# BhavikJoshi/skybox_rt

Measured on AMD Instinct MI355X. Metric: Mrays/sec per GPU + achieved HBM GB/s, 1024^2 primary+shadow tekkaman, higher is better.
Workload: dtype f32

## Files before the change

include/vx_rt.h:

```cpp
#ifndef VX_RT_H
#define VX_RT_H

#include <stdint.h>

#ifdef __cplusplus
extern "C" {
#endif

typedef struct rt_scene* rt_scene_h;
typedef struct rt_renderer* rt_renderer_h;

typedef struct {
  uint32_t num_drawcalls, num_prims, num_geometry, num_layer, num_textures;
  uint32_t bvh_nodes, bvh_tris, bvh_leaves, bvh_depth;
  uint32_t bvh4_nodes, bvh4_depth, bvh4_stack;
  uint32_t bvh4_f16;
  double parse_ms, bvh_ms;
} rt_scene_info_t;

#define RT_RENDER_SHADOWS 0x1u
#define RT_RENDER_PATH 0x8u
#define RT_RENDER_FLAT 0x10u
#define RT_RENDER_RASTER 0x20u
#define RT_RENDER_BVH2 0x40u
// ... 75 lines not shown
int rt_render_kernel_ms(rt_renderer_h r, double* kernel_ms);
int rt_render_run_totals(rt_renderer_h r, double* kernel_ms_sum, uint64_t* timed,
                         uint64_t* launches);
int rt_render_set_timing(rt_renderer_h r, int timed);
int rt_read_framebuffer(rt_renderer_h r, uint32_t* out, uint64_t count);
int rt_read_framebuffer_prev(rt_renderer_h r, uint32_t* out, uint64_t count);

int rt_read_depthbuffer(rt_renderer_h r, uint32_t* out, uint64_t count);

typedef struct {
  uint32_t nodes, depth, launches;
  uint32_t stack4;
  double build_ms;
  double kernel_ms;
  uint32_t nodes4;
  uint32_t depth4;
  uint32_t method;
  uint32_t pad;
} rt_bvh_build_stats_t;
int rt_renderer_build_bvh(rt_renderer_h r, rt_bvh_build_stats_t* stats);
#define RT_BVH_BUILD_LBVH 0u
#define RT_BVH_BUILD_SAH 1u
#define RT_BVH_BUILD_HOST 2u
int rt_renderer_build_bvh_ex(rt_renderer_h r, uint32_t method, rt_bvh_build_stats_t* stats);
int rt_renderer_bvh_stats(rt_renderer_h r, rt_bvh_build_stats_t* stats);
#define RT_BVH_STACK4_UNUSED 0xFFFFFFFFu
int rt_renderer_export_bvh4(rt_renderer_h r, float* nodes4, uint32_t* num_nodes4);
int rt_renderer_export_bvh4h(rt_renderer_h r, void* nodes4h, uint32_t* num_nodes4);
int rt_renderer_export_bvh(rt_renderer_h r, float* nodes, float* tris, uint32_t* num_nodes,
                           uint32_t* num_tris);

int rt_renderer_export_vis_tree(rt_renderer_h r, int32_t* refs, uint32_t* num_nodes,
                                int32_t* leaf_pids, uint32_t* num_leaf);

typedef struct {
  uint32_t device;
  uint32_t launches;
  uint32_t heavy_tiles;
  uint32_t blist_blocks;
  double setup_ms;
  double configure_ms;
  uint64_t blist_entries;
  uint32_t blist_max;
  uint32_t slist_on;
  uint64_t slist_entries;
  uint32_t path_queue;
  uint32_t slist_built;
  uint32_t slist_stale;
  uint32_t lane_grid;
  uint32_t bg_first_chunk;
  uint32_t tier_groups;
  uint64_t btrim_entries;
  uint32_t btrim_blocks;
  uint32_t pad;
} rt_setup_stats_t;
int rt_renderer_setup_stats(rt_renderer_h r, rt_setup_stats_t* stats);

int rt_renderer_set_light(rt_renderer_h r, const float light[3]);
int rt_renderer_set_list_policy(rt_renderer_h r, uint32_t defer_frames);

#define RT_MAX_LIGHTS 16u
int rt_renderer_set_lights(rt_renderer_h r, const float (*lights)[3], uint32_t n);
typedef struct {
  float light[3];
  uint32_t slist_on;
  uint64_t slist_entries;
} rt_light_info_t;
int rt_renderer_lights_info(rt_renderer_h r, rt_light_info_t* out, uint32_t max, uint32_t* n);
int rt_renderer_export_light_lists(rt_renderer_h r, uint32_t light, uint32_t which, void* out, uint64_t bytes,
                                   uint64_t* size);
uint32_t rt_lights_resolve(uint32_t argb, uint32_t occluded, uint32_t k);

#define RT_MAX_PATH_LIGHTS 8u
int rt_renderer_set_path_lights(rt_renderer_h r, const float (*lights)[3], uint32_t n);
uint32_t rt_path_lights_resolve(const uint32_t sums[3], uint32_t k, uint32_t alpha_argb);

#define RT_AOV_GEOM 0x01000000u
#define RT_AOV_SHADOW_RAY 0x02000000u
typedef struct {
  int32_t  pid;
  uint32_t depth_flags;
  float    t;
  uint32_t light_mask;
} rt_aov_t;
int rt_render_aov_start(rt_renderer_h r);
int rt_render_aov(rt_renderer_h r);
int rt_read_aov(rt_renderer_h r, rt_aov_t* out, uint64_t count);
uint32_t rt_aov_relight(uint32_t plain_argb, uint32_t light_mask, uint32_t k);

int rt_relight_capture_start(rt_renderer_h r);
int rt_relight_capture(rt_renderer_h r);
int rt_render_relight_start(rt_renderer_h r, const uint8_t* weights, uint32_t n);
int rt_render_relight(rt_renderer_h r, const uint8_t* weights, uint32_t n);
int rt_read_relight_base(rt_renderer_h r, uint32_t* out, uint64_t count);
uint32_t rt_relight_resolve(uint32_t base_argb, uint32_t depth_flags, uint32_t light_mask, const uint8_t* weights,
                            uint32_t n);

typedef struct {
  int32_t  pid;
  uint32_t depth_flags;
  uint32_t normal;
  uint32_t reserved;
} rt_denoise_guide_t;
typedef struct {
  uint32_t passes;
  uint32_t depth_shift;
  uint32_t color_shift;
// ... 53 lines not shown
```

skybox_rt_amd/csrc/app/rt_app.cpp:

```cpp
#include <dlfcn.h>

#include <algorithm>
#include <cstdio>
#include <cstdlib>
#include <chrono>
#include <map>
#include <cstring>
#include <memory>
#include <string>
#include <vector>

#include "VX_types.h"
#include "app_util.h"
#include "bg_tier.h"
#include "bvh.h"
#include "bvh_common.h"
#include "cgltrace.h"
#include "rt_internal.h"
#include "sah_common.h"
#include "setup_common.h"
#include "setup.h"
#include "vis.h"
#include "vortex.h"
#include "rt_shard.h"
#include "vortex_hip.h"
#include "vx_rt.h"

namespace {

thread_local std::string g_err;

int fail(const std::string& m, int code = -1) {
  g_err = m;
  return code;
}

std::string find_lib_dir() {
  Dl_info info;
  if (dladdr((void*)&find_lib_dir, &info) && info.dli_fname) {
    std::string p(info.dli_fname);
    auto pos = p.rfind('/');
    if (pos != std::string::npos) return p.substr(0, pos);
  }
  return ".";
}

const std::string& lib_dir() {
  static const std::string dir = find_lib_dir();
  return dir;
}

bool file_exists(const std::string& path) {
  FILE* f = std::fopen(path.c_str(), "rb");
  if (f) std::fclose(f);
  return f != nullptr;
}

int upload_image(rt_renderer* r, const std::string& path, vx_buffer_h* out) {
  if (vx_upload_kernel_file(r->dev, path.c_str(), out) == 0) return 0;
  *out = nullptr;
  return fail("cannot upload kernel " + path);
}

int release_idle(rt_renderer* r, vx_buffer_h* buf) {
  if (!*buf) return 0;
  if (vx_ready_wait(r->dev, VX_MAX_TIMEOUT) != 0) return fail("vx_ready_wait failed");
  vx_mem_free(*buf);
  *buf = nullptr;
  return 0;
}
// ... 370 lines not shown
  if (leaf_pids && !r->vis_pids.empty())
    std::memcpy(leaf_pids, r->vis_pids.data(), r->vis_pids.size() * 4);
  return 0;
}

static uint32_t lane_grid_of(rt_renderer* r) {
  if (r->lane_grid_known) return r->lane_grid;
  r->lane_grid_known = true;
  r->lane_grid = 0;
  uint64_t ia = 0;
  uint32_t block = 0, mgrid = 0;
  const vx_buffer_h rt = r->img[rtimg::mode_image(0, 0, r->deep)];
  if (r->lane_chunks > 1 && rt && vx_mem_address(rt, &ia) == 0 &&
      r->launch_shape(r->dev, ia, &block, &mgrid) == 0 && block >= 64) {
    const uint32_t chunks = (r->arg.num_tasks + 63u) / 64u, per = r->lane_chunks * (block / 64u);
    const uint32_t g = std::max(1u, (chunks + per - 1u) / per);
    if (g < mgrid) r->lane_grid = g;
  }
  return r->lane_grid;
}

static uint32_t tier_groups_of(rt_renderer* r, int k, uint32_t grid, bool laned) {
  if (!r->bg_ok || r->bg_mode == 0 || (r->bg_mode == 1 && !laned)) return 0;
  if (r->sl_stale && !r->bg_stale) return 0;
  if (!r->img_shape_known[k]) {
    r->img_shape_known[k] = true;
    uint64_t ia = 0;
    const vx_buffer_h rt = r->img[rtimg::IMG_RT + k];
    if (!(r->launch_shape && rt && vx_mem_address(rt, &ia) == 0 &&
          r->launch_shape(r->dev, ia, &r->img_block[k], &r->img_grid[k]) == 0))
      r->img_block[k] = r->img_grid[k] = 0;
  }
  if (r->img_block[k] < 64 || r->img_grid[k] == 0) return 0;
  if (grid == 0 || grid > r->img_grid[k]) grid = r->img_grid[k];
  const uint32_t chunks = (r->arg.num_tasks + 63u) / 64u;
  return vxtier::tier_groups(vxtier::Config{}, chunks, r->bg_first / vxtier::kChunksPerTile, grid,
                             r->img_block[k] / 64u, r->bg_cost);
}

int rt_renderer_setup_stats(rt_renderer_h r, rt_setup_stats_t* st) {
  if (!r || !st) return fail("null argument");
  if (!r->configured) return fail("renderer not configured");
  if (rtapp::settle_lists(r) != 0) return -1;
  if (r->trim_on && !r->trim_counted) {
    uint32_t c[2] = {0, 0};
    if (vx_copy_from_dev(c, r->btrim_args, RT_BTRIM_ARG_OFFSET + offsetof(rt_btrim_arg_t, stat), sizeof(c)) != 0)
      return fail("vx_copy_from_dev failed");
    r->setup.btrim_entries = c[0];
    r->setup.btrim_blocks = c[1];
    r->trim_counted = true;
  }
  r->setup.slist_on = r->arg.slist_on;
  r->setup.slist_stale = r->sl_stale ? 1u : 0u;
  r->setup.lane_grid = lane_grid_of(r);
  r->setup.bg_first_chunk = r->bg_ok ? r->bg_first : 0u;
  {
    const int k = (r->params.flags & RT_RENDER_INSTRUMENTED) ? 1 : 0;
    r->setup.tier_groups = r->lanes ? tier_groups_of(r, k, r->sl_stale ? 0u : lane_grid_of(r), true)
                                    : tier_groups_of(r, k, 0u, false);
  }
  *st = r->setup;
  return 0;
}

int rt_renderer_set_light(rt_renderer_h r, const float light[3]) {
  if (!r || !light) return fail("null argument");
  if (!r->configured) return fail("renderer not configured");
  if (!(r->params.flags & (RT_RENDER_SHADOWS | RT_RENDER_PATH)) || (r->params.flags & RT_RENDER_RASTER))
    return fail("rt_renderer_set_light: the configuration traces no shadow rays");
  uint32_t launches = 0;
  r->nlights = 0;
  r->relight_n = 0;
  if (rtapp::set_light(r, light, &launches) != 0) return -1;
  r->setup.slist_built = r->sl_mode ? 1u : 0u;
  if (r->accum_on) {
    r->accum_reset = true;
    r->accum_n = 0;
  }
  return 0;
}


static int set_several_lights(rt_renderer_h r, const float (*lights)[3], uint32_t n, rtimg::Group group,
                              const char* who, bool lists, bool need_lists) {
  if (const int e = rtapp::load_images(r, group, who)) return e;
  if (n == 1) {
    const uint32_t defer = r->sl_defer;
    r->sl_defer = 0;
    const int e = rt_renderer_set_light(r, lights[0]);
    r->sl_defer = defer;
    if (e != 0) return e;
    return rtapp::settle_lists(r);
  }
  uint32_t launches = 0;
  if (rtapp::build_light_sets(r, lights, n, lists, &launches) != 0) return -1;
  rt_lights_arg_t la{};
  la.count = n;
  la.slist_n = r->arg.slist_n;
  for (uint32_t i = 0; i < n; ++i) {
    const LightSet& l = r->lsets[i];
    if (need_lists && !l.built)
      return fail(std::string(who) + ": the light-space lists of light " + std::to_string(i) +
                  " do not fit (pt_lights has no BVH shadow walk)", -2);
    std::memcpy(la.l[i].light, l.light, sizeof(l.light));
    la.l[i].slist_on = l.built ? 1u : 0u;
    la.l[i].sidx_addr = l.sidx_addr;
// ... 716 lines not shown
    if (*b) { vx_mem_free(*b); *b = nullptr; }
  if (release_idle(r, &r->accum) != 0) return -1;
  r->accum_on = r->accum_reset = false;
  r->accum_bytes = 0;
  r->accum_n = 0;
  if (release_idle(r, &r->aov) != 0) return -1;
  r->aov_bytes = 0;
  if (release_idle(r, &r->relight_base) != 0) return -1;
  r->relight_base_bytes = 0;
  r->relight_n = 0;
  if (release_idle(r, &r->dn_buf) != 0) return -1;
  r->dn_bytes = 0;
  r->dn_captured = false;
  r->nlights = 0;
  rt_kernel_arg_t& a = r->arg;
  a.width = p->width;
  a.height = p->height;
  uint32_t tlog = RT_TILE_LOG;
  if (raster) {
    tlog = RT_RASTER_TILE_LOG;
    if (const char* e = std::getenv("RT_RASTER_TILE_LOG")) tlog = std::atoi(e) == 5 ? 5u : 4u;
  }
  a.raster_tile_log = tlog;
  a.raster_bin_log = p->tile_logsize ? p->tile_logsize : RT_TILE_LOG;
  if (raster && (a.raster_bin_log < 2 || a.raster_bin_log > 15))
    return fail("tile_logsize must be in [2, 15] (raster_unit.cpp:92)");
  if (!raster && a.raster_bin_log != RT_TILE_LOG)
    return fail("the RT modes bin at RASTER_TILE_LOGSIZE 5; other tile sizes need RT_RENDER_RASTER");
  if ((p->flags & RT_RENDER_COVERAGE) && !raster) return fail("RT_RENDER_COVERAGE needs RT_RENDER_RASTER");
  a.tiles_y = (p->height + (1u << tlog) - 1) >> tlog;
  a.tiles_x = (p->width + (1u << tlog) - 1) >> tlog;
  a.tiles_x_magic = rt_tiles_x_magic(a.tiles_x);
  const uint32_t tiles = a.tiles_x * a.tiles_y;
  r->local_tiles = (tiles > p->shard_index) ? (tiles - p->shard_index + shards - 1) / shards : 0;
  a.num_tasks = r->local_tiles * (raster ? 256u : RT_TILE_PIXELS);
  a.shard_index = p->shard_index;
  a.shard_count = shards;
  a.order_addr = 0;
  a.split_tiles = 0;
  a.split_log = 5;
  a.quad_tiles = 0;
  const bool order_on = !raster && r->local_tiles > 0 &&
                        !(std::getenv("RT_TILE_ORDER") && std::atoi(std::getenv("RT_TILE_ORDER")) == 0);
  bool use_bvh4 = !(p->flags & RT_RENDER_BVH2) && (!r->gpu_bvh || r->gpu_bvh4);
  if (const char* e = std::getenv("RT_BVH_WIDTH")) use_bvh4 = use_bvh4 && std::atoi(e) != 2;
  r->use_bvh4 = use_bvh4;
  a.flags = ((p->flags & RT_RENDER_SHADOWS) ? RT_FLAG_SHADOWS : 0u) |
            ((p->flags & RT_RENDER_PATH) ? RT_FLAG_PATH : 0u) |
            ((p->flags & RT_RENDER_FLAT) ? RT_FLAG_FLAT : 0u) |
            (raster ? RT_FLAG_RASTER : 0u) |
            ((p->flags & RT_RENDER_COVERAGE) ? RT_FLAG_COVERAGE : 0u) |
            (s->tie_high ? RT_FLAG_TIE_HIGH : 0u) | (compact ? RT_FLAG_COMPACT : 0u) |
            (use_bvh4 ? RT_FLAG_BVH4 : 0u) |
            (use_bvh4 && (r->gpu_bvh || !s->bvh.nodes4h.empty()) ? RT_FLAG_BVH4H : 0u);
  if (tail && s->geometry.size() > 0 && !(a.flags & RT_FLAG_BVH4H))
    return fail("a scene with an ordered tail needs the binary16 BVH4; this tree needs the generic (deep) "
                "images, which have no output-merger variant (use RT_RENDER_RASTER)", -2);
  if (!raster && !tail && !(p->flags & RT_RENDER_FLAT) && !(a.flags & RT_FLAG_BVH4H) && !r->deep &&
      load_deep_images(r) != 0)
    return -1;
  const char* pqe = std::getenv("RT_PT_QUEUE");
  r->pq = (p->flags & RT_RENDER_PATH) && !r->generic_tree() && r->img[rtimg::IMG_PT_PRIMARY] &&
          r->launch_group && pqe && std::atoi(pqe) == 1;
  a.bounces = p->bounces;
  a.seed = p->seed;
  a.clear_color = p->clear_color;
  a.sx = 2.0f / (float)p->width;
  a.sy = 2.0f / (float)p->height;
  a.light[0] = p->light[0];
  a.light[1] = p->light[1];
  a.light[2] = p->light[2];
  const uint64_t npx = compact ? (uint64_t)r->local_tiles * RT_TILE_PIXELS
                                  : (uint64_t)p->width * p->height;
  r->cbuf_bytes = npx * 4;
  const char* sv = std::getenv("RT_SETUP");
  const char* vt = std::getenv("RT_VIS_TREE");
  const bool device = !(p->flags & RT_RENDER_HOST_SETUP) && !(sv && std::string(sv) == "host") &&
                      !(!raster && vt && std::string(vt) == "screen");
  uint32_t heavy = 0, launches = 0;
  const char* bl = std::getenv("RT_BLOCK_LISTS");
  const bool bvh_walk = (p->flags & RT_RENDER_BVH_WALK) != 0;
  const bool lists = !raster && !(p->flags & RT_RENDER_FLAT) && !(bl && std::atoi(bl) == 0) && !bvh_walk &&
                     a.num_geom > 0 && r->local_tiles > 0;
  a.blist_blocks = 0;
  a.blist_addr = a.bidx_addr = 0;
  a.cdesc_addr = 0;
  a.cdesc_first = 0;
  r->cdesc_n = 0;
  r->setup.blist_entries = 0;
  r->setup.blist_max = 0;
  const char* bte = std::getenv("RT_BLIST_TRIM");
  const bool trim = lists && !(p->flags & RT_RENDER_INSTRUMENTED) && !(bte && std::atoi(bte) == 0);
  r->trim_on = r->trim_counted = false;
  r->setup.btrim_entries = 0;
  r->setup.btrim_blocks = 0;
  const char* sle = std::getenv("RT_SHADOW_LISTS");
  const bool slists = device && !raster && !(p->flags & RT_RENDER_FLAT) &&
                      (p->flags & (RT_RENDER_SHADOWS | RT_RENDER_PATH)) && a.num_geom > 0 &&
                      !(sle && std::atoi(sle) == 0) && !bvh_walk;
  r->sl_mode = slists;
  r->sl_stale = false;
  a.slist_on = 0;
  r->setup.slist_entries = 0;
  const auto t1 = std::chrono::steady_clock::now();
  if (device) {
    r->vis_refs.clear();
    r->vis_pids.clear();
// ... 1048 lines not shown
```

skybox_rt_amd/csrc/kernels/rt_common.h:

```cpp
#pragma once

#include <stdint.h>

#ifndef RT_BLOCK_THREADS
#define RT_BLOCK_THREADS 64
#endif
#define RT_STACK_SHALLOW 24
#define RT_STACK_DEEP 32
#ifndef RT_MAX_STACK
#define RT_MAX_STACK RT_STACK_SHALLOW
#endif
#ifndef RT_PUSH_UNCOND
#define RT_PUSH_UNCOND 0
#endif
#define RT_STACK_ROWS (RT_MAX_STACK + (RT_PUSH_UNCOND ? 3 : 0))
#define RT_TILE_LOG 5
#define RT_TILE_PIXELS 1024
#define RT_RASTER_TILE_LOG 4

#define RT_FLAG_SHADOWS  0x1u
#define RT_FLAG_TIE_HIGH 0x2u
#define RT_FLAG_COMPACT  0x4u
#define RT_FLAG_PATH     0x8u
#define RT_FLAG_FLAT     0x10u
#define RT_FLAG_RASTER   0x20u
#define RT_FLAG_BVH4     0x40u
#define RT_FLAG_BVH4H    0x80u
#define RT_FLAG_COVERAGE 0x100u

#define RT_LW_LIGHT    0x1u
#define RT_LW_NO_SLIST 0x2u
#define RT_LW_CBUF_MASK 0xffffff00u
#define RT_LW_ACCUM_RESET   0x4u
#define RT_LW_ACCUM_K_SHIFT 3
#define RT_LW_ACCUM_K_MASK  0xf8u
#define RT_ACCUM_MAX_K      32u
#define RT_ACCUM_MAX_SAMPLES (1u << 24)

#define RT_DC_DEPTH   0x1u
#define RT_DC_COLOR   0x2u
#define RT_DC_TEX     0x4u
#define RT_DC_MODULATE 0x8u

#define RT_LEAF_FLAG 0x80000000u
#define RT_EMPTY_REF (-1)

#define RT_MPM_USER 3
enum {
  RT_STAT_PRIMARY = 0, RT_STAT_SHADOW, RT_STAT_HITS, RT_STAT_OCCLUDED,
  RT_STAT_NODE_VISITS, RT_STAT_TRI_TESTS, RT_STAT_LAYER_TESTS, RT_STAT_SHADED,
  RT_STAT_TEXEL_BYTES, RT_STAT_BOUNCE, RT_STAT_RECT_TESTS, RT_STAT_EDGE_TESTS, RT_STAT_COUNT = 16
};

typedef struct { float v[16]; } rt_node_t;

typedef struct { float v[32]; } rt_node4_t;

typedef struct { uint16_t b[24]; int32_t child[4]; } rt_node4h_t;


typedef struct { float v[12]; } rt_tri_t;

#define RT_VIS_EMPTY_RECT 0x0000ffffu
#define RT_VIS_ZMIN_NONE 0xffffffffu
typedef struct {
  uint32_t lo[4], hi[4], zmin[4];
  int32_t child[4];
} rt_vnode_t;
typedef struct {
  int32_t edges[9];
  uint32_t rx, ry;
  int32_t pid;
  int32_t z[3];
  uint32_t zmin;
} rt_vtri_t;

typedef struct {
  int32_t edges[3][3];
  int32_t attribs[7][3];
  uint32_t dc;
  uint32_t pad;
// ... 260 lines not shown
```

skybox_rt_amd/csrc/kernels/rt_kernel.hip:

```cpp
#include <hip/hip_runtime.h>

#ifndef RT_BLOCK_THREADS
#define RT_BLOCK_THREADS 64
#endif
#define VX_BLOCK_THREADS RT_BLOCK_THREADS
#include "rt_trace.h"

#ifndef RT_LIGHTS
#define RT_LIGHTS 0
#endif
#ifndef RT_PATHQ
#define RT_PATHQ 0
#endif
#ifndef RT_BG_TIER
#define RT_BG_TIER 0
#endif
#ifndef RT_BG_LAYERS
#define RT_BG_LAYERS 0
#endif
#if RT_BG_LAYERS && !RT_BG_TIER
#error "RT_BG_LAYERS is for the background tier"
#endif
#if RT_BG_LAYERS && !defined(RT_INSTRUMENT) && !RT_LIGHTS
#define RT_BG_TABLE 1
#else
#define RT_BG_TABLE 0
#endif
#if RT_LIGHTS && (RT_PATHQ || RT_BVH_WALK || !RT_ONLY_BVH4H)
#error "RT_LIGHTS is for the primary+shadow list image on the binary16 BVH4"
#endif
#if RT_BG_TIER && (RT_PATHQ || RT_BVH_WALK || !RT_CHUNK_DESC)
#error "RT_BG_TIER is for the primary+shadow list image with the chunk descriptor table"
#endif

namespace {

using namespace rtk;

constexpr int kWaves = RT_BLOCK_THREADS / 64;

#define RT_QUEUE 128
#define RT_LANE_STACK (!RT_ONLY_BVH4H)
struct WaveLds {
#if RT_LANE_STACK
  int32_t stack[RT_STACK_ROWS][64];
#define RT_WSTACK(w, lane) (&(w).stack[0][(lane)])
#else
#define RT_WSTACK(w, lane) ((int32_t*)nullptr)
#endif
  uint32_t q_out[RT_QUEUE];
  uint32_t q_xy[RT_QUEUE];
  float q_t[RT_QUEUE];
  int32_t q_pid[RT_QUEUE];
  uint32_t q_color[RT_QUEUE];
  uint32_t q_count;
};

__device__ __forceinline__ void kernel_body(const vx_task_t& task, const Scene& S, WaveLds& w,
                                            Counters& cnt) {
  const uint32_t t = task.blockIdx.x;
  const uint32_t c = (uint32_t)__builtin_amdgcn_readfirstlane(t) >> 6;
  uint32_t x, y, out;
#if RT_CHUNK_DESC && !RT_BVH_WALK
  uint2 oc = make_uint2(0u, 0u);
  if (S.cdesc != 0 && c >= S.cdesc_first) {
    const uint4 d = S.A.sld_u4(S.cdesc + 16u * (c - S.cdesc_first));
    uint32_t ln = t & 63u;
    asm volatile("" : "+v"(ln));
    x = (d.x & 0xffffu) + (ln & 7u);
    y = (d.x >> 16) + (ln >> 3);
    out = d.y + (ln >> 3) * (d.w >> 16) + (ln & 7u);
    oc = make_uint2(d.z, d.w & 0xffffu);
  } else {
    const ChunkMap cm = chunk_map(S, task_args(S), c);
    uint32_t cx, cy, co;
    chunk_pixel(S, cm, t & 63u, &cx, &cy, &co);
    x = cx;
    y = cy;
    out = co;
    if (S.blist_blocks) oc = block_header(S, (cm.lt << 4) | cm.blk);
  }
#else
  const ChunkMap cm = chunk_map(S, task_args(S), c);
  chunk_pixel(S, cm, t & 63u, &x, &y, &out);
  const uint32_t lb = (cm.lt << 4) | cm.blk;
#endif
  const bool in = x < S.width && y < S.height;
  cnt.primary += in;
  const bool tie_high = (S.flags & RT_FLAG_TIE_HIGH) != 0;
#ifdef RT_STAMPS
  if (lane_id() == 0) __vx_mpm_lds[3] = (uint32_t)__builtin_amdgcn_s_memrealtime();
#endif
#if RT_CHUNK_DESC && !RT_BVH_WALK
  int32_t hit;
  if (S.blist_blocks) {
    hit = block_primary(S, oc, x, y, in, tie_high, cnt);
  } else {
    const int32_t h = trace_primary_packet(walk_scene(S), x, y, in, tie_high, cnt);
    hit = in ? h : -1;
  }
#else
  const int32_t hit = trace_primary(S, lb, x, y, in, tie_high, cnt);
#endif
#ifdef RT_STAMPS
  if (lane_id() == 0) __vx_mpm_lds[14] = (uint32_t)__builtin_amdgcn_s_memrealtime();
#endif
  cnt.hits += hit >= 0;
  const int32_t spid = resolve_layers(S, x, y, in && hit < 0, hit, cnt);
#ifdef RT_STAMPS
  if (lane_id() == 0) __vx_mpm_lds[4] = (uint32_t)__builtin_amdgcn_s_memrealtime();
#endif
  uint32_t color = shade_wave(S, spid, x, y, S.clear_color, cnt);
#ifdef RT_STAMPS
  if (lane_id() == 0) __vx_mpm_lds[11] = (uint32_t)__builtin_amdgcn_s_memrealtime();
#endif
  Ray r;
  primary_dir(S, x, y, r);
  const float th = hit >= 0 ? plane_t(S, r, hit) : 0.0f;
#if RT_PATHQ
  const bool path = hit >= 0 && secondary_ok(th);
  pathq_append(S, path, t, th, hit, color);
  if (in && !path) store_out(S, out, color);
  (void)w;
  return;
#endif
  const bool shadow = hit >= 0 && secondary_ok(th) && (rt_usgpr(S.flags) & RT_FLAG_SHADOWS) != 0;
  const uint64_t m = __ballot(shadow);
  if (m) {
    const uint32_t base = w.q_count;
    if (shadow) {
      const uint32_t rank = __builtin_amdgcn_mbcnt_hi(
          (uint32_t)(m >> 32), __builtin_amdgcn_mbcnt_lo((uint32_t)m, 0u));
      const uint32_t slot = base + rank;
      w.q_out[slot] = out;
      w.q_xy[slot] = x | (y << 16);
      w.q_t[slot] = th;
      w.q_pid[slot] = hit;
      w.q_color[slot] = color;
    }
    __builtin_amdgcn_wave_barrier();
    if (lane_id() == 0) w.q_count = base + (uint32_t)__popcll(m);
    __builtin_amdgcn_wave_barrier();
  }
  if (in && !shadow) store_out(S, out, color);
#ifdef RT_STAMPS
  if (lane_id() == 0) __vx_mpm_lds[5] = (uint32_t)__builtin_amdgcn_s_memrealtime();
#endif
}

__device__ __forceinline__ void shadow_drain(bool final, const Scene& S, WaveLds& w,
                                             Counters& cnt) {
#ifdef RT_STAMPS
  if (final && lane_id() == 0) __vx_mpm_lds[15] = (uint32_t)__builtin_amdgcn_s_memrealtime();
  if (final && lane_id() == 0) __vx_mpm_lds[8] = w.q_count;
  if (!final && w.q_count >= 64 && lane_id() == 0)
    __vx_mpm_lds[6] = (uint32_t)__builtin_amdgcn_s_memrealtime();
#endif
  if (!(rt_usgpr(S.flags) & RT_FLAG_SHADOWS)) return;
  const uint32_t lane = lane_id();
  uint32_t n = w.q_count;
  const bool tie_high = (S.flags & RT_FLAG_TIE_HIGH) != 0;
  while (n >= 64 || (final && n > 0)) {
    const uint32_t take = n < 64 ? n : 64;
    const uint32_t base = n - take;
    const bool active = lane < take;
    const uint32_t slot = base + lane;
    const uint32_t xy = w.q_xy[slot];
// ... 112 lines not shown
#else
      const int32_t spid = resolve_layers(S, x, y, in, -1, cnt);
      const uint32_t color = shade_wave(S, spid, x, y, S.clear_color, cnt);
#endif
      if (in) store_out(S, out, color);
      ++ran;
    }
  }
  vx_mpm_add(VX_MPM_TASKS, ran);
  flush(RT_STAT_PRIMARY, cnt.primary);
#ifdef RT_INSTRUMENT
  flush(RT_STAT_LAYER_TESTS, cnt.layer_tests);
  flush(RT_STAT_SHADED, cnt.shaded);
  flush(RT_STAT_TEXEL_BYTES, cnt.texel_bytes);
#endif
}
#endif

}

#if !defined(RT_WAVES_PER_EU) && RT_ONLY_BVH4H
#if RT_BVH_WALK
#define RT_WAVES_PER_EU 5
#else
#define RT_WAVES_PER_EU 7
#endif
#endif
#ifdef RT_WAVES_PER_EU
VX_MAIN_OCC(rt_kernel_arg_t, arg, RT_BLOCK_THREADS, RT_WAVES_PER_EU) {
#else
VX_MAIN(rt_kernel_arg_t, arg, RT_BLOCK_THREADS) {
#endif
#if RT_BG_TIER
  if (vx_launch_tag != 0 && blockIdx.x >= vx_launch_tag) {
    bg_tier(arg, vx_launch_tag, vx_launch_words);
    return 0;
  }
#endif
  __shared__ WaveLds s_wave[kWaves];
  WaveLds& w = s_wave[threadIdx.x >> 6];
#ifdef RT_STAMPS
  const uint64_t t_stamp0 = __builtin_amdgcn_s_memrealtime();
#endif
  Counters cnt;
  Scene S = load_scene(arg, vx_launch_words);
#ifdef RT_STAMPS
  if (threadIdx.x == 0) __vx_mpm_lds[10] = (uint32_t)__builtin_amdgcn_s_memrealtime();
#endif
  if ((threadIdx.x & 63u) == 0) w.q_count = 0;
  __builtin_amdgcn_wave_barrier();
#if RT_BG_TIER
  const uint32_t tier_wgs = vx_launch_tag != 0 ? vx_launch_tag : gridDim.x;
  const uint32_t tier_end = vx_launch_tag != 0 ? bg_first_chunk(arg) : 0xffffffffu;
  const int rc = vx_spawn_chunks_ex(
      S.num_tasks, 0u, tier_end, blockIdx.x * kWaves + (threadIdx.x >> 6), tier_wgs * kWaves,
      [&](const vx_task_t& task, const Scene* s) { kernel_body(task, *s, w, cnt); },
      [&](bool final, const Scene* s) { shadow_drain(final, *s, w, cnt); }, &S);
#else
  const int rc = vx_spawn_tasks_ex(
      S.num_tasks,
      [&](const vx_task_t& task, const Scene* s) { kernel_body(task, *s, w, cnt); },
      [&](bool final, const Scene* s) { shadow_drain(final, *s, w, cnt); }, &S);
#endif
#ifdef RT_STAMPS
  if (threadIdx.x == 0) {
    __vx_mpm_lds[12] = (uint32_t)t_stamp0;
    __vx_mpm_lds[13] = (uint32_t)__builtin_amdgcn_s_memrealtime();
  }
#endif
#ifndef RT_STAMPS
  flush_rays(cnt);
#endif
#ifdef RT_INSTRUMENT
  flush(RT_STAT_NODE_VISITS, cnt.visits);
  flush(RT_STAT_TRI_TESTS, cnt.tests);
  flush(RT_STAT_LAYER_TESTS, cnt.layer_tests);
  flush(RT_STAT_SHADED, cnt.shaded);
  flush(RT_STAT_TEXEL_BYTES, cnt.texel_bytes);
#endif
  return rc;
}
```

skybox_rt_amd/csrc/kernels/rt_trace.h:

```cpp
#pragma once

#include <hip/hip_runtime.h>

#include "gfx_device.h"
#include "rt_common.h"
#include "vx_spawn.h"

#ifndef RT_ONLY_BVH4H
#define RT_ONLY_BVH4H 0
#endif
#ifndef RT_BVH_WALK
#define RT_BVH_WALK 0
#endif
#ifndef RT_SHADE_KEY
#define RT_SHADE_KEY 0
#endif
#ifndef RT_LEAN_SCENE
#define RT_LEAN_SCENE 0
#endif
#ifndef RT_UTEST
#define RT_UTEST 0
#endif
#ifndef RT_CHUNK_DESC
#define RT_CHUNK_DESC 0
// ... 572 lines not shown
        {
          uint4 tw[3 * H];
          RT_LD_BEGIN();
          S.A.sld_u4n<3 * H>(S.tris + 48u * (first + q0), tw);
          RT_LD_END(1);
#pragma unroll
          for (uint32_t j = 0; j < H; ++j) {
            ta[j] = u4f(tw[3 * j]); tb[j] = u4f(tw[3 * j + 1]); tc[j] = u4f(tw[3 * j + 2]);
          }
        }
#pragma unroll
        for (uint32_t j = 0; j < H; ++j) {
          if (q0 + j < count) {
            RT_CNT(cnt.tests += (uint32_t)(live_m >> lane) & 1u;)
            float t;
            const bool hit = mt_hit_bf(r, ta[j], tb[j], tc[j], 0.0f, &t) && t < tmax &&
                             __float_as_int(ta[j].w) != skip;
            const uint64_t m = __ballot(hit) & live_m;
            done_m |= m;
            live_m &= ~m;
          }
        }
      }
      if ((act_m & ~done_m) == 0) break;
    }
    if (sp == 0) break;
    --sp;
    const uint32_t lo = (uint32_t)__builtin_amdgcn_readlane(vmlo, sp);
    const uint32_t hi = (uint32_t)__builtin_amdgcn_readlane(vmhi, sp);
    live_m = (((uint64_t)hi << 32) | lo) & ~done_m;
    ref = __builtin_amdgcn_readlane(vstk, sp);
  }
  return act && ((done_m >> lane_id()) & 1u);
}

__device__ __forceinline__ uint32_t slist_cell(const Ray& s, uint32_t N) {
  const float u0 = -s.d[0], u1 = -s.d[1], u2 = -s.d[2];
  int k = 0;
  float m = fabsf(u0);
  if (fabsf(u1) > m) { k = 1; m = fabsf(u1); }
  if (fabsf(u2) > m) { k = 2; m = fabsf(u2); }
  if (!(m > 0.0f)) return 0u;
  const float uk = k == 0 ? u0 : (k == 1 ? u1 : u2);
  const float ui = k == 0 ? u1 : u0, uj = k == 2 ? u1 : u2;
  const int f = 2 * k + (uk < 0.0f ? 1 : 0);
  const float hn = (float)N * 0.5f;
  const int cx = min(max((int)floorf((ui / m + 1.0f) * hn), 0), (int)N - 1);
  const int cy = min(max((int)floorf((uj / m + 1.0f) * hn), 0), (int)N - 1);
  return ((uint32_t)f * N + (uint32_t)cy) * N + (uint32_t)cx;
}
__device__ __forceinline__ float slist_limit(const Ray& s) {
  return (s.d[0] * s.d[0] + s.d[1] * s.d[1] + s.d[2] * s.d[2]) * 1.001f;
}
__device__ __forceinline__ bool occluded_list(const Scene& S, const Ray& s, bool act, int32_t skip,
                                              Counters& cnt, uint32_t sidx, uint32_t slist, uint32_t slist_n) {
  if (!act) return false;
  const uint32_t cell = slist_cell(s, slist_n);
  const uint32_t off = S.A.ld_u32(sidx + 8u * cell), n = S.A.ld_u32(sidx + 8u * cell + 4u);
  const float lim = slist_limit(s);
  uint32_t o = slist + 48u * off;
  for (uint32_t q = 0; q < n; q += 2, o += 96u) {
    float4 t[6];
#pragma unroll
    for (int w = 0; w < 6; ++w) t[w] = S.A.ld_f4(o + 16u * w);
#pragma unroll
    for (int e = 0; e < 2; ++e) {
      if (q + e >= n) break;
      if (t[3 * e + 1].w > lim) return false;
      RT_CNT(++cnt.tests;)
      float th;
      if (__float_as_int(t[3 * e].w) != skip && mt_hit(s, t[3 * e], t[3 * e + 1], t[3 * e + 2], 0.0f, &th) &&
          th < 1.0f)
        return true;
    }
  }
  return false;
}
__device__ __forceinline__ bool occluded_list(const Scene& S, const Ray& s, bool act, int32_t skip,
                                              Counters& cnt) {
  return occluded_list(S, s, act, skip, cnt, S.sidx, S.slist, S.slist_n);
}

__device__ __forceinline__ uint32_t xpart(uint32_t v, bool hi) {
  (void)hi;
  return (uint32_t)__builtin_amdgcn_update_dpp(0, (int)v, 0xB1, 0xF, 0xF, false);
}
__device__ __forceinline__ float xpartf(float v, bool hi) {
  return __uint_as_float(xpart(__float_as_uint(v), hi));
}
__device__ __forceinline__ uint32_t xlow(uint32_t v) {
  return (uint32_t)__builtin_amdgcn_update_dpp(0, (int)v, 0xA0, 0xF, 0xF, false);
}
__device__ __forceinline__ float xlowf(float v) { return __uint_as_float(xlow(__float_as_uint(v))); }

struct CoopHalf {
  uint32_t w[6];
  uint2 cc;
};
__device__ __forceinline__ CoopHalf coop_half_load(const Scene& S, uint32_t ref, bool hi) {
  const uint32_t no = S.nodes4 + 128u * S.num_nodes4 + 64u * ref;
  const uint32_t hb = no + (hi ? 4u : 0u);
  CoopHalf h;
#pragma unroll
  for (int i = 0; i < 6; ++i) h.w[i] = S.A.ld_u32(hb + 8u * i);
  h.cc = S.A.ld_u2(no + 48u + (hi ? 8u : 0u));
  return h;
}
template <bool SCALAR>
__device__ __forceinline__ int32_t node4_coop(const Scene& S, uint32_t ref, const Ray& r, float lim,
                                              bool hi, int32_t* mem, int& sp,
                                              const CoopHalf* pre = nullptr) {
  auto ld = [&](uint32_t o) { return SCALAR ? S.A.sld_f4(o) : S.A.ld_f4(o); };
  const uint32_t no = S.nodes4 + 128u * S.num_nodes4 + 64u * ref;
  auto h2 = [](float w, float& a, float& b) {
    const uint32_t u = __float_as_uint(w);
    a = (float)__builtin_bit_cast(_Float16, (uint16_t)(u & 0xffffu));
    b = (float)__builtin_bit_cast(_Float16, (uint16_t)(u >> 16));
  };
  float lx[2], hx[2], ly[2], hy[2], lz[2], hz[2];
  int32_t c[2];
  if (!SCALAR) {
    const CoopHalf hh = pre ? *pre : coop_half_load(S, ref, hi);
    const auto f = [&](int i) { return __uint_as_float(hh.w[i]); };
    h2(f(0), lx[0], lx[1]); h2(f(1), hx[0], hx[1]);
    h2(f(2), ly[0], ly[1]); h2(f(3), hy[0], hy[1]);
    h2(f(4), lz[0], lz[1]); h2(f(5), hz[0], hz[1]);
    c[0] = (int32_t)hh.cc.x; c[1] = (int32_t)hh.cc.y;
  } else {
    const float4 px = ld(no), py = ld(no + 16), pz = ld(no + 32), cf = ld(no + 48);
// ... 448 lines not shown
  const uint32_t pp = px > 0xffffu ? 0xffffffffu : px | (py << 16);
  uint32_t bz = VX_OM_DEPTH_MASK;
  int32_t bpid = -1;
  uint4 e[2];
  S.A.sld_u4n<2>(S.blist + 16u * oc.x, e);
  for (uint32_t k = 0; k < oc.y; k += 2) {
    if (__ballot(rect2_in(e[0].y, e[0].z, pp) && e[0].w <= bz) == 0) break;
    uint4 r0[4], r1[4], en[2];
    S.A.sld_u4n<4>(S.vgeom + 64u * e[0].x, r0);
    S.A.sld_u4n<4>(S.vgeom + 64u * e[1].x, r1);
    S.A.sld_u4n<2>(S.blist + 16u * (oc.x + k + 2), en);
#ifdef RT_INSTRUMENT
    cnt.tests += lane_id() == 0 ? (k + 1 < oc.y ? 2u : 1u) : 0u;
#endif
    vis_test(r0[0], r0[1], r0[2], r0[3], px, py, tie_high, bz, bpid);
    if (k + 1 < oc.y) vis_test(r1[0], r1[1], r1[2], r1[3], px, py, tie_high, bz, bpid);
    e[0] = en[0];
    e[1] = en[1];
  }
  return act ? bpid : -1;
}
__device__ __forceinline__ int32_t block_primary_z(const Scene& S, uint2 oc, uint32_t px, uint32_t py,
                                                   bool act, bool tie_high, Counters& cnt, uint32_t* bzo) {
  (void)cnt;
  if (!act) px = 0xffffffffu;
  const uint32_t pp = px > 0xffffu ? 0xffffffffu : px | (py << 16);
  uint32_t bz = VX_OM_DEPTH_MASK;
  int32_t bpid = -1;
  uint4 e[2];
  S.A.sld_u4n<2>(S.blist + 16u * oc.x, e);
  for (uint32_t k = 0; k < oc.y; k += 2) {
    if (__ballot(rect2_in(e[0].y, e[0].z, pp) && e[0].w <= bz) == 0) break;
    uint4 r0[4], r1[4], en[2];
    S.A.sld_u4n<4>(S.vgeom + 64u * e[0].x, r0);
    S.A.sld_u4n<4>(S.vgeom + 64u * e[1].x, r1);
    S.A.sld_u4n<2>(S.blist + 16u * (oc.x + k + 2), en);
    vis_test(r0[0], r0[1], r0[2], r0[3], px, py, tie_high, bz, bpid);
    if (k + 1 < oc.y) vis_test(r1[0], r1[1], r1[2], r1[3], px, py, tie_high, bz, bpid);
    e[0] = en[0];
    e[1] = en[1];
  }
  *bzo = act ? bz : VX_OM_DEPTH_MASK;
  return act ? bpid : -1;
}

__device__ __forceinline__ int32_t trace_primary(const Scene& S, uint32_t lb, uint32_t px, uint32_t py,
                                                 bool act, bool tie_high, Counters& cnt) {
  if (!RT_BVH_WALK && rt_usgpr(S.blist_blocks))
    return block_primary(S, block_header(S, lb), px, py, act, tie_high, cnt);
  const int32_t h = trace_primary_packet(walk_scene(S), px, py, act, tie_high, cnt);
  return act ? h : -1;
}

__device__ __forceinline__ float plane_t(const Scene& S, const Ray& r, int32_t pid) {
  const uint32_t o = S.ptris + 48u * (uint32_t)pid;
  const float4 a = S.A.ld_f4(o), b = S.A.ld_f4(o + 16), c = S.A.ld_f4(o + 32);
  const float e1[3] = {b.x, b.y, b.z}, e2[3] = {c.x, c.y, c.z};
  float pvec[3], tvec[3], qvec[3];
  cross3(pvec, r.d, e2);
  const float det = dot3(e1, pvec);
  tvec[0] = r.o[0] - a.x;
  tvec[1] = r.o[1] - a.y;
  tvec[2] = r.o[2] - a.z;
  cross3(qvec, tvec, e1);
  return dot3(e2, qvec) / det;
}
__device__ __forceinline__ bool secondary_ok(float t) { return t > 0.0f && t < INFINITY; }

__device__ __forceinline__ int32_t resolve_layers_n(const Scene& S, uint32_t px, uint32_t py, bool need,
                                                    int32_t spid, uint32_t* tests) {
  uint64_t pend = __ballot(need);
  const uint32_t lead = lane_id() == (uint32_t)__builtin_ctzll(__ballot(1)) ? 1u : 0u;
  for (uint32_t k = 0; pend != 0 && k < S.num_layer; ++k) {
    uint4 lw[3];
    S.A.sld_u4n<3>(S.vlayers + 64u * k, lw);
    const uint4 A = lw[0], B = lw[1], C = lw[2];
    const bool mine = (pend & (1ull << lane_id())) != 0;
    *tests += lead;
    bool f = false;
    if (mine && rect_in(C.y, px) && rect_in(C.z, py)) {
      const int32_t e0[3] = {(int32_t)A.x, (int32_t)A.y, (int32_t)A.z};
      const int32_t e1[3] = {(int32_t)A.w, (int32_t)B.x, (int32_t)B.y};
      const int32_t e2[3] = {(int32_t)B.z, (int32_t)B.w, (int32_t)C.x};
      f = gfx::edge_eval(e0, px, py) >= 0 && gfx::edge_eval(e1, px, py) >= 0 &&
          gfx::edge_eval(e2, px, py) >= 0;
    }
    if (f) spid = (int32_t)C.w;
    pend &= ~__ballot(f);
  }
  return spid;
}
__device__ __forceinline__ int32_t resolve_layers(const Scene& S, uint32_t px, uint32_t py, bool need,
                                                  int32_t spid, Counters& cnt) {
  uint32_t tests = 0;
  spid = resolve_layers_n(S, px, py, need, spid, &tests);
#ifdef RT_INSTRUMENT
  cnt.layer_tests += tests;
#else
  (void)cnt;
#endif
  return spid;
}

__device__ __forceinline__ void tile_xy(uint32_t gt, uint32_t tiles_x, uint32_t magic, uint32_t* tx,
                                        uint32_t* ty) {
  uint32_t q = __umulhi(gt, magic);
  int32_t r = (int32_t)(gt - q * tiles_x);
  if (r < 0) {
    --q;
    r += (int32_t)tiles_x;
  } else if (r >= (int32_t)tiles_x) {
    ++q;
    r -= (int32_t)tiles_x;
  }
  *tx = (uint32_t)r;
  *ty = q;
}
struct TaskPix {
// ... 217 lines not shown
```

skybox_rt_amd/rt.py:

```python
from __future__ import annotations

import ctypes as C
import os

import numpy as np

from . import _lib

RT_RENDER_SHADOWS = 0x1
RT_RENDER_PATH = 0x8
RT_RENDER_FLAT = 0x10
RT_RENDER_RASTER = 0x20
RT_RENDER_BVH2 = 0x40
PT_SEED = 0x5EED
RT_RENDER_INSTRUMENTED = 0x100
RT_RENDER_COMPACT = 0x200
RT_RENDER_COUNTERS = 0x400
RT_RENDER_HOST_SETUP = 0x800
RT_RENDER_BVH_WALK = 0x2000
RT_SCENE_OM_LAYERS = 0x1
RECORDS = {"prims": (0, np.int32, 32), "bbox": (1, np.uint32, 2), "vis": (2, np.uint32, 4),
           "vnodes": (3, np.uint32, 16), "vtris": (4, np.int32, 16), "vlayers": (5, np.int32, 16),
           "vgeom": (6, np.int32, 16), "order": (7, np.uint32, 1), "ptris": (8, np.float32, 12),
           "geom": (9, np.float32, 12), "bidx": (10, np.uint32, 2), "blist": (11, np.uint32, 4),
           "cdesc": (14, np.uint32, 4), "cdesc_host": (15, np.uint32, 4),
           "sidx": (12, np.uint32, 2), "slist": (13, np.float32, 12),
           "oidx": (16, np.uint32, 2), "olist": (17, np.uint32, 1),
           "bglayer": (18, np.uint32, 2), "bglayer_host": (19, np.uint32, 2),
           "btidx": (20, np.uint32, 2), "btrim": (21, np.uint32, 4),
           "btidx_host": (22, np.uint32, 2), "btrim_host": (23, np.uint32, 4)}
RT_BVH_STACK4_UNUSED = 0xFFFFFFFF
RT_BVH_BUILD_HOST = 2
CLEAR_COLOR = 0xFF000000
DEFAULT_LIGHT = (0.0, 60.0, 80.0)
TILE = 32


class SceneInfo(C.Structure):
    _fields_ = [(n, C.c_uint32) for n in (
        "num_drawcalls", "num_prims", "num_geometry", "num_layer", "num_textures",
        "bvh_nodes", "bvh_tris", "bvh_leaves", "bvh_depth", "bvh4_nodes", "bvh4_depth",
        "bvh4_stack", "bvh4_f16")] + [
        ("parse_ms", C.c_double), ("bvh_ms", C.c_double)]


class BvhBuildStats(C.Structure):
    _fields_ = [("nodes", C.c_uint32), ("depth", C.c_uint32), ("launches", C.c_uint32),
                ("stack4", C.c_uint32), ("build_ms", C.c_double), ("kernel_ms", C.c_double),
                ("nodes4", C.c_uint32), ("depth4", C.c_uint32), ("method", C.c_uint32),
                ("pad", C.c_uint32)]

    def as_dict(self):
        return {n: getattr(self, n) for n, _ in self._fields_ if n != "pad"}


class SetupStats(C.Structure):
    _fields_ = [("device", C.c_uint32), ("launches", C.c_uint32), ("heavy_tiles", C.c_uint32),
                ("blist_blocks", C.c_uint32), ("setup_ms", C.c_double), ("configure_ms", C.c_double),
                ("blist_entries", C.c_uint64), ("blist_max", C.c_uint32), ("slist_on", C.c_uint32),
                ("slist_entries", C.c_uint64), ("path_queue", C.c_uint32), ("slist_built", C.c_uint32),
                ("slist_stale", C.c_uint32), ("lane_grid", C.c_uint32),
                ("bg_first_chunk", C.c_uint32), ("tier_groups", C.c_uint32),
                ("btrim_entries", C.c_uint64), ("btrim_blocks", C.c_uint32), ("pad", C.c_uint32)]

    def as_dict(self):
        return {n: getattr(self, n) for n, _ in self._fields_ if n != "pad"}


class LightInfo(C.Structure):
    _fields_ = [("light", C.c_float * 3), ("slist_on", C.c_uint32), ("slist_entries", C.c_uint64)]


RT_MAX_LIGHTS = 16
RT_MAX_PATH_LIGHTS = 8
AOV_DTYPE = np.dtype([("pid", "<i4"), ("depth_flags", "<u4"), ("t", "<f4"), ("light_mask", "<u4")])
DENOISE_GUIDE_DTYPE = np.dtype([("pid", "<i4"), ("depth_flags", "<u4"), ("normal", "<u4"), ("reserved", "<u4")])
DENOISE_PASSES, DENOISE_DEPTH_SHIFT, DENOISE_COLOR_SHIFT = 2, 2, 3
RT_AOV_DEPTH_MASK = 0xFFFFFF
RT_AOV_GEOM = 0x01000000
RT_AOV_SHADOW_RAY = 0x02000000


class RenderParams(C.Structure):
    _fields_ = [("width", C.c_uint32), ("height", C.c_uint32), ("flags", C.c_uint32),
                ("light", C.c_float * 3), ("clear_color", C.c_uint32),
                ("shard_index", C.c_uint32), ("shard_count", C.c_uint32),
                ("bounces", C.c_uint32), ("seed", C.c_uint32), ("tile_logsize", C.c_uint32)]


class Stats(C.Structure):
    _fields_ = [(n, C.c_uint64) for n in (
        "primary_rays", "shadow_rays", "geometry_hits", "occluded", "node_visits",
        "tri_tests", "layer_tests", "shaded", "texel_bytes", "tasks")] + [
        ("kernel_ms", C.c_double), ("grid", C.c_uint32), ("block", C.c_uint32),
        ("num_tasks", C.c_uint32), ("local_tiles", C.c_uint32), ("bounce_rays", C.c_uint64),
        ("rect_tests", C.c_uint64), ("edge_tests", C.c_uint64)]

    def as_dict(self):
        return {n: getattr(self, n) for n, _ in self._fields_}


class RtError(RuntimeError):
    pass


_h = None


def lib():
    global _h
    if _h is None:
        h = _lib.load("librtapp.so")
        vp, u32, u64 = C.c_void_p, C.c_uint32, C.c_uint64
        sig = {
            "rt_scene_load": [C.c_char_p, C.POINTER(vp)],
            "rt_scene_load_ex": [C.c_char_p, u32, u32, u32, C.POINTER(vp)],
# ... 595 lines not shown
```

Baseline: 137,000.

## Fuse the shadow-list test into the primary body for each wave's final chunk

Adds a chunk scheduler that tells the kernel body when it is processing a wave's last chunk. For that chunk, the shadow-list test runs inline instead of going through the deferred shadow drain. The hit triangle's plane record and the shadow-list cell header are loaded early, before shading, so their latency overlaps with the shading work. The aim is to shorten the tail where a wave drains queued shadow rays with little work left, at the cost of another kernel variant, extra registers and new env and flag plumbing.

Result: faster. 141,600, median of 6 (+3.3%).

```diff
diff --git a/include/vx_rt.h b/include/vx_rt.h
--- a/include/vx_rt.h
+++ b/include/vx_rt.h
@@ -151,7 +151,7 @@
   uint32_t tier_groups;
   uint64_t btrim_entries;
   uint32_t btrim_blocks;
-  uint32_t pad;
+  uint32_t fused_chunk;
 } rt_setup_stats_t;
 int rt_renderer_setup_stats(rt_renderer_h r, rt_setup_stats_t* stats);
 
diff --git a/skybox_rt_amd/csrc/app/fused_chunk.h b/skybox_rt_amd/csrc/app/fused_chunk.h
--- /dev/null
+++ b/skybox_rt_amd/csrc/app/fused_chunk.h
@@ -0,0 +1,21 @@
+#pragma once
+#include <cstdint>
+#include <cstdlib>
+
+namespace rtfused {
+
+inline bool knob(const char* env) { return !(env && *env && std::atoi(env) == 0); }
+
+struct Conf {
+  bool shadows;
+  bool path, flat, raster;
+  bool tail;
+};
+
+inline uint32_t flag(const Conf& c, const char* env, uint32_t bit) {
+  if (!knob(env)) return 0u;
+  if (!c.shadows || c.path || c.flat || c.raster || c.tail) return 0u;
+  return bit;
+}
+
+}
diff --git a/skybox_rt_amd/csrc/app/rt_app.cpp b/skybox_rt_amd/csrc/app/rt_app.cpp
--- a/skybox_rt_amd/csrc/app/rt_app.cpp
+++ b/skybox_rt_amd/csrc/app/rt_app.cpp
@@ -16,6 +16,7 @@
 #include "bvh.h"
 #include "bvh_common.h"
 #include "cgltrace.h"
+#include "fused_chunk.h"
 #include "rt_internal.h"
 #include "sah_common.h"
 #include "setup_common.h"
@@ -492,6 +493,7 @@
   }
   r->setup.slist_on = r->arg.slist_on;
   r->setup.slist_stale = r->sl_stale ? 1u : 0u;
+  r->setup.fused_chunk = (r->arg.flags & RT_FLAG_FUSED) ? 1u : 0u;
   r->setup.lane_grid = lane_grid_of(r);
   r->setup.bg_first_chunk = r->bg_ok ? r->bg_first : 0u;
   {
@@ -1314,7 +1316,10 @@
             ((p->flags & RT_RENDER_COVERAGE) ? RT_FLAG_COVERAGE : 0u) |
             (s->tie_high ? RT_FLAG_TIE_HIGH : 0u) | (compact ? RT_FLAG_COMPACT : 0u) |
             (use_bvh4 ? RT_FLAG_BVH4 : 0u) |
-            (use_bvh4 && (r->gpu_bvh || !s->bvh.nodes4h.empty()) ? RT_FLAG_BVH4H : 0u);
+            (use_bvh4 && (r->gpu_bvh || !s->bvh.nodes4h.empty()) ? RT_FLAG_BVH4H : 0u) |
+            rtfused::flag({(p->flags & RT_RENDER_SHADOWS) != 0, (p->flags & RT_RENDER_PATH) != 0,
+                           (p->flags & RT_RENDER_FLAT) != 0, raster, tail},
+                          std::getenv("RT_FUSED_CHUNK"), RT_FLAG_FUSED);
   if (tail && s->geometry.size() > 0 && !(a.flags & RT_FLAG_BVH4H))
     return fail("a scene with an ordered tail needs the binary16 BVH4; this tree needs the generic (deep) "
                 "images, which have no output-merger variant (use RT_RENDER_RASTER)", -2);
diff --git a/skybox_rt_amd/csrc/kernels/rt_common.h b/skybox_rt_amd/csrc/kernels/rt_common.h
--- a/skybox_rt_amd/csrc/kernels/rt_common.h
+++ b/skybox_rt_amd/csrc/kernels/rt_common.h
@@ -27,6 +27,7 @@
 #define RT_FLAG_BVH4     0x40u
 #define RT_FLAG_BVH4H    0x80u
 #define RT_FLAG_COVERAGE 0x100u
+#define RT_FLAG_FUSED    0x200u
 
 #define RT_LW_LIGHT    0x1u
 #define RT_LW_NO_SLIST 0x2u
diff --git a/skybox_rt_amd/csrc/kernels/rt_kernel.hip b/skybox_rt_amd/csrc/kernels/rt_kernel.hip
--- a/skybox_rt_amd/csrc/kernels/rt_kernel.hip
+++ b/skybox_rt_amd/csrc/kernels/rt_kernel.hip
@@ -25,6 +25,12 @@
 #define RT_BG_TABLE 1
 #else
 #define RT_BG_TABLE 0
+#endif
+#ifndef RT_FUSED_CHUNK
+#define RT_FUSED_CHUNK 0
+#endif
+#if RT_FUSED_CHUNK && (RT_LIGHTS || RT_PATHQ || RT_BVH_WALK || !RT_ONLY_BVH4H)
+#error "RT_FUSED_CHUNK is for the one-light primary+shadow list image on the binary16 BVH4"
 #endif
 #if RT_LIGHTS && (RT_PATHQ || RT_BVH_WALK || !RT_ONLY_BVH4H)
 #error "RT_LIGHTS is for the primary+shadow list image on the binary16 BVH4"
@@ -56,14 +62,106 @@
   uint32_t q_count;
 };
 
+#if RT_FUSED_CHUNK
+struct ChunkPlace {
+  bool last;
+};
+template <typename F, typename E, typename Arg>
+__device__ __forceinline__ int spawn_chunks_placed(uint32_t num_tasks, uint32_t c1, uint32_t w, uint32_t nw,
+                                                   F kernel_func, E epilogue, Arg* arg) {
+  __vx_declare_tasks(num_tasks);
+  const uint32_t nchunks = (num_tasks + VX_CHUNK - 1) / VX_CHUNK;
+  if (c1 > nchunks) c1 = nchunks;
+  uint32_t ran = 0;
+  vx_task_t task;
+  task.threadIdx.x = task.threadIdx.y = task.threadIdx.z = 0;
+  task.blockIdx.y = task.blockIdx.z = 0;
+  for (uint32_t c = (uint32_t)__builtin_amdgcn_readfirstlane(w); c < c1; c += nw) {
+    const uint32_t t = c * VX_CHUNK + (threadIdx.x & 63u);
+    if (t < num_tasks) {
+      task.task_id = t;
+      task.blockIdx.x = t;
+      ChunkPlace cp;
+      cp.last = c + nw >= c1;
+      kernel_func(task, cp, arg);
+      ++ran;
+    }
+    if (c + nw < c1) epilogue(false, arg);
+  }
+  epilogue(true, arg);
+  vx_mpm_add(VX_MPM_TASKS, ran);
+  return 0;
+}
+
+struct FusedRay {
+  float o[3], d[3];
+  uint2 hd;
+};
+struct PlaneRec {
+  float4 a, b, c;
+};
+__device__ __forceinline__ PlaneRec fused_planes(const Scene& S, int32_t hit) {
+  PlaneRec P;
+  P.a = P.b = P.c = make_float4(0.0f, 0.0f, 0.0f, 0.0f);
+  if (hit >= 0) {
+    const uint32_t o = S.ptris + 48u * (uint32_t)hit;
+    P.a = S.A.ld_f4(o);
+    P.b = S.A.ld_f4(o + 16);
+    P.c = S.A.ld_f4(o + 32);
+  }
+  return P;
+}
+__device__ __forceinline__ FusedRay fused_header(const Scene& S, uint32_t x, uint32_t y, int32_t hit,
+                                                 const PlaneRec& P, Counters& cnt) {
+  FusedRay f;
+  Ray r, s;
+  primary_dir(S, x, y, r);
+  const float th = hit >= 0 ? plane_t(r, P.a, P.b, P.c) : 0.0f;
+  const bool shadow = hit >= 0 && secondary_ok(th);
+  shadow_ray(S, r, th, s);
+  f.hd = make_uint2(0u, 0u);
+  if (shadow) f.hd = S.A.ld_u2(S.sidx + 8u * slist_cell(s, S.slist_n));
+#pragma unroll
+  for (int k = 0; k < 3; ++k) {
+    f.o[k] = s.o[k];
+    f.d[k] = s.d[k];
+  }
+  cnt.shadow += shadow;
+  return f;
+}
+__device__ __forceinline__ void fused_verdict(const Scene& S, uint32_t x, uint32_t y, uint32_t out, bool in,
+                                              int32_t hit, FusedRay f, uint32_t color, Counters& cnt) {
+  if (f.hd.y != 0u) {
+    Ray s;
+#pragma unroll
+    for (int k = 0; k < 3; ++k) {
+      s.o[k] = f.o[k];
+      s.d[k] = f.d[k];
+    }
+    if (slist_scan(S, s, hit, cnt, S.slist, f.hd.x, f.hd.y)) {
+      ++cnt.occluded;
+      color = shadowed(color);
+    }
+  }
+  if (in) store_out(S, out, color);
+}
+#endif
+
+#if RT_FUSED_CHUNK
+#define RT_BODY_DEAL , const ChunkPlace &cp
+#define RT_BODY_U(v) rt_usgpr(v)
+#else
+#define RT_BODY_DEAL
+#define RT_BODY_U(v) (v)
+#endif
 __device__ __forceinline__ void kernel_body(const vx_task_t& task, const Scene& S, WaveLds& w,
-                                            Counters& cnt) {
+                                            Counters& cnt RT_BODY_DEAL) {
   const uint32_t t = task.blockIdx.x;
   const uint32_t c = (uint32_t)__builtin_amdgcn_readfirstlane(t) >> 6;
   uint32_t x, y, out;
 #if RT_CHUNK_DESC && !RT_BVH_WALK
   uint2 oc = make_uint2(0u, 0u);
-  if (S.cdesc != 0 && c >= S.cdesc_first) {
+  if (RT_BODY_U(S.cdesc) != 0 && c >= S.cdesc_first) {
     const uint4 d = S.A.sld_u4(S.cdesc + 16u * (c - S.cdesc_first));
     uint32_t ln = t & 63u;
     asm volatile("" : "+v"(ln));
@@ -78,7 +176,7 @@
     x = cx;
     y = cy;
     out = co;
-    if (S.blist_blocks) oc = block_header(S, (cm.lt << 4) | cm.blk);
+    if (RT_BODY_U(S.blist_blocks)) oc = block_header(S, (cm.lt << 4) | cm.blk);
   }
 #else
   const ChunkMap cm = chunk_map(S, task_args(S), c);
@@ -87,13 +185,13 @@
 #endif
   const bool in = x < S.width && y < S.height;
   cnt.primary += in;
-  const bool tie_high = (S.flags & RT_FLAG_TIE_HIGH) != 0;
+  const bool tie_high = (RT_BODY_U(S.flags) & RT_FLAG_TIE_HIGH) != 0;
 #ifdef RT_STAMPS
   if (lane_id() == 0) __vx_mpm_lds[3] = (uint32_t)__builtin_amdgcn_s_memrealtime();
 #endif
 #if RT_CHUNK_DESC && !RT_BVH_WALK
   int32_t hit;
-  if (S.blist_blocks) {
+  if (RT_BODY_U(S.blist_blocks)) {
     hit = block_primary(S, oc, x, y, in, tie_high, cnt);
   } else {
     const int32_t h = trace_primary_packet(walk_scene(S), x, y, in, tie_high, cnt);
@@ -106,13 +204,32 @@
   if (lane_id() == 0) __vx_mpm_lds[14] = (uint32_t)__builtin_amdgcn_s_memrealtime();
 #endif
   cnt.hits += hit >= 0;
+#if RT_FUSED_CHUNK
+  const bool fused = (rt_usgpr(S.flags) & (RT_FLAG_FUSED | RT_FLAG_SHADOWS)) == (RT_FLAG_FUSED | RT_FLAG_SHADOWS) &&
+                     rt_usgpr(S.slist_on) && cp.last;
+  PlaneRec P;
+  if (fused) P = fused_planes(S, hit);
+#endif
   const int32_t spid = resolve_layers(S, x, y, in && hit < 0, hit, cnt);
 #ifdef RT_STAMPS
   if (lane_id() == 0) __vx_mpm_lds[4] = (uint32_t)__builtin_amdgcn_s_memrealtime();
 #endif
+#if RT_FUSED_CHUNK
+  FusedRay fr;
+  if (fused) fr = fused_header(S, x, y, hit, P, cnt);
+#endif
   uint32_t color = shade_wave(S, spid, x, y, S.clear_color, cnt);
 #ifdef RT_STAMPS
   if (lane_id() == 0) __vx_mpm_lds[11] = (uint32_t)__builtin_amdgcn_s_memrealtime();
+#endif
+#if RT_FUSED_CHUNK
+  if (fused) {
+    fused_verdict(S, x, y, out, in, hit, fr, color, cnt);
+#ifdef RT_STAMPS
+    if (lane_id() == 0) __vx_mpm_lds[5] = (uint32_t)__builtin_amdgcn_s_memrealtime();
+#endif
+    return;
+  }
 #endif
   Ray r;
   primary_dir(S, x, y, r);
@@ -331,6 +448,19 @@
 #if RT_BG_TIER
   const uint32_t tier_wgs = vx_launch_tag != 0 ? vx_launch_tag : gridDim.x;
   const uint32_t tier_end = vx_launch_tag != 0 ? bg_first_chunk(arg) : 0xffffffffu;
+#endif
+#if RT_FUSED_CHUNK
+#if RT_BG_TIER
+  const uint32_t deal_w = blockIdx.x * kWaves + (threadIdx.x >> 6), deal_nw = tier_wgs * kWaves, deal_end = tier_end;
+#else
+  const uint32_t deal_w = __vx_logical_block() * kWaves + (threadIdx.x >> 6), deal_nw = gridDim.x * kWaves,
+                 deal_end = 0xffffffffu;
+#endif
+  const int rc = spawn_chunks_placed(
+      S.num_tasks, deal_end, deal_w, deal_nw,
+      [&](const vx_task_t& task, const ChunkPlace& cp, const Scene* s) { kernel_body(task, *s, w, cnt, cp); },
+      [&](bool final, const Scene* s) { shadow_drain(final, *s, w, cnt); }, &S);
+#elif RT_BG_TIER
   const int rc = vx_spawn_chunks_ex(
       S.num_tasks, 0u, tier_end, blockIdx.x * kWaves + (threadIdx.x >> 6), tier_wgs * kWaves,
       [&](const vx_task_t& task, const Scene* s) { kernel_body(task, *s, w, cnt); },
diff --git a/skybox_rt_amd/csrc/kernels/rt_trace.h b/skybox_rt_amd/csrc/kernels/rt_trace.h
--- a/skybox_rt_amd/csrc/kernels/rt_trace.h
+++ b/skybox_rt_amd/csrc/kernels/rt_trace.h
@@ -648,11 +648,8 @@
 __device__ __forceinline__ float slist_limit(const Ray& s) {
   return (s.d[0] * s.d[0] + s.d[1] * s.d[1] + s.d[2] * s.d[2]) * 1.001f;
 }
-__device__ __forceinline__ bool occluded_list(const Scene& S, const Ray& s, bool act, int32_t skip,
-                                              Counters& cnt, uint32_t sidx, uint32_t slist, uint32_t slist_n) {
-  if (!act) return false;
-  const uint32_t cell = slist_cell(s, slist_n);
-  const uint32_t off = S.A.ld_u32(sidx + 8u * cell), n = S.A.ld_u32(sidx + 8u * cell + 4u);
+__device__ __forceinline__ bool slist_scan(const Scene& S, const Ray& s, int32_t skip, Counters& cnt,
+                                           uint32_t slist, uint32_t off, uint32_t n) {
   const float lim = slist_limit(s);
   uint32_t o = slist + 48u * off;
   for (uint32_t q = 0; q < n; q += 2, o += 96u) {
@@ -671,6 +668,13 @@
     }
   }
   return false;
+}
+__device__ __forceinline__ bool occluded_list(const Scene& S, const Ray& s, bool act, int32_t skip,
+                                              Counters& cnt, uint32_t sidx, uint32_t slist, uint32_t slist_n) {
+  if (!act) return false;
+  const uint32_t cell = slist_cell(s, slist_n);
+  const uint32_t off = S.A.ld_u32(sidx + 8u * cell), n = S.A.ld_u32(sidx + 8u * cell + 4u);
+  return slist_scan(S, s, skip, cnt, slist, off, n);
 }
 __device__ __forceinline__ bool occluded_list(const Scene& S, const Ray& s, bool act, int32_t skip,
                                               Counters& cnt) {
@@ -1225,9 +1229,7 @@
   return act ? h : -1;
 }
 
-__device__ __forceinline__ float plane_t(const Scene& S, const Ray& r, int32_t pid) {
-  const uint32_t o = S.ptris + 48u * (uint32_t)pid;
-  const float4 a = S.A.ld_f4(o), b = S.A.ld_f4(o + 16), c = S.A.ld_f4(o + 32);
+__device__ __forceinline__ float plane_t(const Ray& r, const float4& a, const float4& b, const float4& c) {
   const float e1[3] = {b.x, b.y, b.z}, e2[3] = {c.x, c.y, c.z};
   float pvec[3], tvec[3], qvec[3];
   cross3(pvec, r.d, e2);
@@ -1237,6 +1239,10 @@
   tvec[2] = r.o[2] - a.z;
   cross3(qvec, tvec, e1);
   return dot3(e2, qvec) / det;
+}
+__device__ __forceinline__ float plane_t(const Scene& S, const Ray& r, int32_t pid) {
+  const uint32_t o = S.ptris + 48u * (uint32_t)pid;
+  return plane_t(r, S.A.ld_f4(o), S.A.ld_f4(o + 16), S.A.ld_f4(o + 32));
 }
 __device__ __forceinline__ bool secondary_ok(float t) { return t > 0.0f && t < INFINITY; }
 
diff --git a/skybox_rt_amd/rt.py b/skybox_rt_amd/rt.py
--- a/skybox_rt_amd/rt.py
+++ b/skybox_rt_amd/rt.py
@@ -61,7 +61,7 @@
                 ("slist_entries", C.c_uint64), ("path_queue", C.c_uint32), ("slist_built", C.c_uint32),
                 ("slist_stale", C.c_uint32), ("lane_grid", C.c_uint32),
                 ("bg_first_chunk", C.c_uint32), ("tier_groups", C.c_uint32),
-                ("btrim_entries", C.c_uint64), ("btrim_blocks", C.c_uint32), ("pad", C.c_uint32)]
+                ("btrim_entries", C.c_uint64), ("btrim_blocks", C.c_uint32), ("fused_chunk", C.c_uint32)]
 
     def as_dict(self):
         return {n: getattr(self, n) for n, _ in self._fields_ if n != "pad"}
```
